# LockedFlysher/optimal_control_problem

Hardware: NVIDIA B200
Metric: batched OCP SQP solves/sec (H=20) (higher is better)
Workload: dtype f64

## Files before the change

optimal_control_problem_b200/csrc/admm_common.cuh:

```cuda
#pragma once

#include <cuda_runtime.h>
#include <stdint.h>
#include <stdio.h>

#include "ocp_b200.h"

namespace ocpb200 {

constexpr double kInfty = 1e30, kMinScaling = 1e-4, kMaxScaling = 1e4;
constexpr double kRhoMin = 1e-6, kRhoMax = 1e6, kRhoTol = 1e-4, kRhoEqOverIneq = 1e3;
constexpr double kDivisionTol = 1e-30;
constexpr int kRedWidth = 16;
constexpr int kMaxWarps = 32;

typedef uint16_t idx_t;

#ifdef OCP_B200_CANARY
constexpr int kCanaryDoubles = 2;
#else
constexpr int kCanaryDoubles = 0;
#endif
__device__ __forceinline__ double canary_value(int id) { return __longlong_as_double(0x7ff4dead00000000LL + id); }

struct KRun { uint16_t ka, kc, len, row0; };
struct KEntry {
  uint32_t dest0, dest1;
  int32_t ppos;
  uint32_t run_begin;
  uint16_t nruns, diag;
  uint32_t pad;
};

struct PatternDev {
  int n, m, nnz_a, nnz_p, nnz_h;
  int nblk, minv_doubles, max_bs;
  int n_long, n_short;
  int tri_ok, tri_np, tri_bs, tri_nb, tri_ld;
  int stage_slots;
  int kprog_entries;
  const KEntry* kprog;
  const KRun* kruns;
  int idx_entries;
  const idx_t* idx_base;
  const idx_t* a_colptr;
  const idx_t* a_rowidx;
  const idx_t* a_rowptr;
  const idx_t* a_colidx;
  const idx_t* a_perm;
  const idx_t* p_colptr;
  const idx_t* p_rowidx;
  const int* p_src;
  const idx_t* blk_ptr;
  const idx_t* blk_of_col;
  const int* minv_off;
  const idx_t* rows_long;
  const idx_t* rows_short;
};

struct SolveArgs {
  int B;
  const double* h_vals; int ld_h;
  const double* q; int ld_n;
  const double* a_vals; int ld_a;
  const double* l; const double* u; int ld_m;
  double* sol_x;
  double* sol_y;
  double* info;
  double* x_iter; int np; int N; double sqp_alpha;
  double* stats; int first_step;
  double* trace; int max_trace; int* n_trace;
  long long* phase;
  int* counter;
  double* slab; size_t slab_doubles;
};

struct Reducer {
  double* buf;
  int parity;
  int half;
};

template <int NV, bool kMax>
__device__ __forceinline__ void block_reduce(double (&v)[NV], Reducer& R) {
  const int lane = threadIdx.x & 31, warp = threadIdx.x >> 5, nw = blockDim.x >> 5;
#pragma unroll
  for (int k = 0; k < NV; ++k) {
    double a = v[k];
#pragma unroll
    for (int o = 16; o > 0; o >>= 1) {
      const double b = __shfl_xor_sync(0xffffffffu, a, o);
      a = kMax ? fmax(a, b) : a + b;
    }
    v[k] = a;
  }
  double* buf = R.buf + R.parity * R.half;
  R.parity ^= 1;
  if (lane == 0) {
#pragma unroll
    for (int k = 0; k < NV; ++k) buf[warp * NV + k] = v[k];
  }
  __syncthreads();
#pragma unroll
  for (int k = 0; k < NV; ++k) {
    double a = buf[k];
    for (int w = 1; w < nw; ++w) a = kMax ? fmax(a, buf[w * NV + k]) : a + buf[w * NV + k];
    v[k] = a;
  }
}

__device__ __forceinline__ double limit_scaling(double v) {
  v = v < kMinScaling ? 1.0 : v;
  return v > kMaxScaling ? kMaxScaling : v;
}

template <typename F>
__device__ __forceinline__ void for_rows_A(const PatternDev& P, const double* __restrict__ Aval,
                                           const double* __restrict__ src, F f) {
  const int tid = threadIdx.x, T = blockDim.x;
  for (int base = 0; base < P.n_long; base += (T >> 2)) {
    const int idx = base + (tid >> 2);
    const bool valid = idx < P.n_long;
    double s = 0.0;
    int row = 0;
    if (valid) {
      row = P.rows_long[idx];
      const int e = P.a_rowptr[row + 1];
#pragma unroll 4
      for (int k = P.a_rowptr[row] + (tid & 3); k < e; k += 4) s += Aval[P.a_perm[k]] * src[P.a_colidx[k]];
    }
    s += __shfl_xor_sync(0xffffffffu, s, 1);
    s += __shfl_xor_sync(0xffffffffu, s, 2);
    if (valid && (tid & 3) == 0) f(row, s);
  }
  for (int idx = tid; idx < P.n_short; idx += T) {
    const int row = P.rows_short[idx];
    double s = 0.0;
    const int e = P.a_rowptr[row + 1];
#pragma unroll 4
    for (int k = P.a_rowptr[row]; k < e; ++k) s += Aval[P.a_perm[k]] * src[P.a_colidx[k]];
    f(row, s);
  }
}

__device__ __forceinline__ double col_dot_A(const PatternDev& P, const double* __restrict__ Aval,
                                            const double* __restrict__ v, int j) {
  double s = 0.0;
  const int e = P.a_colptr[j + 1];
#pragma unroll 4
  for (int k = P.a_colptr[j]; k < e; ++k) s += Aval[k] * v[P.a_rowidx[k]];
  return s;
}
__device__ __forceinline__ double col_dot_P(const PatternDev& P, const double* __restrict__ Pval,
                                            const double* __restrict__ v, int j) {
  double s = 0.0;
  const int e = P.p_colptr[j + 1];
#pragma unroll 4
  for (int k = P.p_colptr[j]; k < e; ++k) s += Pval[k] * v[P.p_rowidx[k]];
  return s;
}

struct PhaseClock {
  long long* out; long long t0;
  __device__ PhaseClock(long long* o) : out((blockIdx.x == 0 && threadIdx.x == 0) ? o : nullptr), t0(0) { if (out) t0 = clock64(); }
  __device__ __forceinline__ void lap(int phase) {
    if (out) { const long long t = clock64(); out[phase] += t - t0; t0 = t; }
  }
};


#ifdef OCP_B200_FINE_PHASES
#define OCP_B200_FINE_CLOCK(name, ptr) PhaseClock name(ptr)
#define OCP_B200_FINE_LAP(name, phase) name.lap(phase)
#else
#define OCP_B200_FINE_CLOCK(name, ptr)
#define OCP_B200_FINE_LAP(name, phase)
#endif

struct QpResult {
  int status, iters, pcg_iters, rho_updates, checks;
  double prim_res, dual_res, rho;
};

__device__ inline void write_outputs(const PatternDev& P, const SolveArgs& A, const double* xs, const double* ys,
                                      Reducer& R, int inst, const QpResult& res) {
  const bool solved_setup = res.status != OCP_B200_QP_UNSOLVED || res.iters > 0;
  if (A.sol_x)
    for (int j = threadIdx.x; j < P.n; j += blockDim.x) A.sol_x[size_t(inst) * P.n + j] = solved_setup ? xs[j] : 0.0;
  if (A.sol_y)
    for (int i = threadIdx.x; i < P.m; i += blockDim.x) A.sol_y[size_t(inst) * P.m + i] = solved_setup ? ys[i] : 0.0;
  double nrm[1] = {0.0};
  if (A.x_iter) {
    double* xi = A.x_iter + size_t(inst) * A.N;
    for (int i = threadIdx.x; i < A.N; i += blockDim.x) {
      const double dx = solved_setup ? A.sqp_alpha * xs[A.np + i] : 0.0;
      xi[i] += dx;
      nrm[0] += dx * dx;
    }
    block_reduce<1, false>(nrm, R);
  }
  if (threadIdx.x == 0) {
    if (A.info) {
      double* f = A.info + size_t(inst) * OCP_B200_NINFO;
      f[OCP_B200_INFO_STATUS] = res.status; f[OCP_B200_INFO_ITERS] = res.iters;
      f[OCP_B200_INFO_PCG_ITERS] = res.pcg_iters; f[OCP_B200_INFO_PRIM_RES] = res.prim_res;
      f[OCP_B200_INFO_DUAL_RES] = res.dual_res; f[OCP_B200_INFO_RHO] = res.rho;
      f[OCP_B200_INFO_RHO_UPDATES] = res.rho_updates; f[OCP_B200_INFO_CHECKS] = res.checks;
    }
    if (A.stats) {
      double* s = A.stats + size_t(inst) * OCP_B200_NSTATS;
      if (A.first_step) for (int k = 0; k < OCP_B200_NSTATS; ++k) s[k] = 0.0;
      s[OCP_B200_STAT_QP_STATUS] = res.status;
      s[OCP_B200_STAT_SQP_STEPS] += 1.0;
      s[OCP_B200_STAT_ADMM_ITERS] += res.iters;
      s[OCP_B200_STAT_PCG_ITERS] += res.pcg_iters;
      s[OCP_B200_STAT_PRIM_RES] = res.prim_res;
      s[OCP_B200_STAT_DUAL_RES] = res.dual_res;
      s[OCP_B200_STAT_RHO_UPDATES] += res.rho_updates;
      s[OCP_B200_STAT_LAST_ADMM] = res.iters;
      s[OCP_B200_STAT_LAST_RHO] = res.rho;
      s[OCP_B200_STAT_CHECKS] += res.checks;
      s[OCP_B200_STAT_STEP_NORM] = sqrt(nrm[0]);
    }
  }
  __syncthreads();
}

}
```

optimal_control_problem_b200/csrc/admm_compact_kernel.cuh:

```cuda
#pragma once

#include "admm_direct_kernel.cuh"
#include "periodic_index.h"

namespace ocpb200 {
namespace compact {

using direct::Rho;
using direct::Work;

constexpr int kMaxGuards = 40;
struct Layout {
  int nguard;
  size_t guard_off[kMaxGuards];
  bool guard_slab[kMaxGuards];
  size_t b, x, w, z, y, vend;
  size_t aval, ctype, dp, xp, piv, arena, smem_doubles;
  size_t rscale, psm;
  size_t dp2, s, sp, stage, fb;
  int s_stride, sp_stride, stage_stride;
  size_t dinv, lsub, lp, q, l, u, D, E, pval, dx, dy, an, cn, sx, sz, sy, slab_doubles;
  bool ok, q_smem, lu_smem, scale_smem;
};

// ... 215 lines not shown
}

template <int BS>
__device__ inline void tri_solve_twisted_tmem(const PatternDev& P, const Work& W, uint32_t tmem) {
  const int tid = threadIdx.x, T = blockDim.x, lane = tid & 31, warp = tid >> 5;
  const int np = P.tri_np, nb = P.tri_nb, N = nb * BS;
  constexpr int ld = BS + 2;
  const int mid = nb / 2;
  double* bx = W.b + np;
  OCP_B200_FINE_CLOCK(clk, W.phase);
  const uint32_t base = tmem + (static_cast<uint32_t>(32 * (warp & 3)) << 16);
  double Lj[8];
  if (warp < 2) run_chain_tmem<BS, false>(W, bx, sweep_chain(warp, nb), base, lane);
  if (warp == 0 && mid + 1 < nb) slab_block_part<BS, false>(W.Lsub, mid + 1, lane, Lj);
  __syncthreads();
  if (warp == 0 && mid + 1 < nb) direct::sweep_stage<BS>(Lj, bx + (mid + 1) * BS + (lane & 1) * 8, bx + mid * BS + (lane >> 1), (lane & 1) == 0);
  __syncthreads();
  OCP_B200_FINE_LAP(clk, OCP_B200_PHASE_SOLVE_FWD);
  if (np > 0) {
    const int nw = T >> 5;
    if (direct::border_rows_by_warp(np, N, nw)) {
      direct::border_rows_dispatch(W.Lp, bx, W.b, W.xp, N, warp, lane, nw);
    } else {
    const int hw = tid >> 4, hl = tid & 15, nhw = T >> 4;
    for (int r0 = 0; r0 < np; r0 += nhw) {
      const int r = r0 + hw;
      const bool have = r < np;
      const double* rowp = W.Lp + size_t(have ? r : 0) * N;
      double s0 = 0.0, s1 = 0.0;
      for (int j0 = hl; j0 < N; j0 += 128) {
        double lv[8], yv[8];
#pragma unroll
        for (int u = 0; u < 8; ++u) {
          const int j = j0 + 16 * u;
          const bool ok = have && j < N;
          lv[u] = ok ? rowp[j] : 0.0;
          yv[u] = ok ? bx[j] : 0.0;
        }
#pragma unroll
        for (int u = 0; u < 8; u += 2) { s0 = fma(lv[u], yv[u], s0); s1 = fma(lv[u + 1], yv[u + 1], s1); }
      }
      double s = s0 + s1;
#pragma unroll
      for (int o = 8; o > 0; o >>= 1) s += __shfl_xor_sync(0xffffffffu, s, o);
      if (have && hl == 0) W.xp[r] = W.b[r] - s;
    }
    }
    __syncthreads();
    direct::border_apply_inverse(W.Dp, W.xp, W.b, np, tid);
    __syncthreads();
  }
  OCP_B200_FINE_LAP(clk, OCP_B200_PHASE_SOLVE_BORDER);
  {
#ifndef OCP_B200_DIAG_PASSES
#define OCP_B200_DIAG_PASSES 1
#endif
    constexpr int kPass = OCP_B200_DIAG_PASSES;
    const int Tb = (T / BS) * BS;
    const int k1 = tid / BS, r1 = tid % BS, kstep = T / BS;
    for (int base0 = 0, k0 = k1; base0 < N; base0 += kPass * Tb, k0 += kPass * kstep) {
      double vq[kPass];
#pragma unroll
      for (int q = 0; q < kPass; ++q) {
        const int base_j = base0 + q * Tb, k = k0 + q * kstep;
        const int j = tid < Tb ? base_j + tid : N;
        double v = 0.0;
        if (j < N) {
          {
            const double2* d2 = reinterpret_cast<const double2*>(W.Dinv + size_t(k) * BS * ld + r1 * ld);
            const double* yk = bx + k * BS;
            double dr[BS];
#pragma unroll
            for (int t = 0; t < BS / 2; ++t) { const double2 x = d2[t]; dr[2 * t] = x.x; dr[2 * t + 1] = x.y; }
            double s0 = 0.0, s1 = 0.0, s2 = 0.0, s3 = 0.0;
#pragma unroll
            for (int t = 0; t < BS; t += 4) {
              s0 = fma(dr[t], yk[t], s0); s1 = fma(dr[t + 1], yk[t + 1], s1);
              s2 = fma(dr[t + 2], yk[t + 2], s2); s3 = fma(dr[t + 3], yk[t + 3], s3);
            }
            v = (s0 + s1) + (s2 + s3);
          }
          double v1 = 0.0;
          if (np == 12) {
            double lv[12];
#pragma unroll
            for (int p = 0; p < 12; ++p) lv[p] = W.Lp[size_t(p) * N + j];
#pragma unroll
            for (int p = 0; p < 12; p += 2) { v = fma(-lv[p], W.b[p], v); v1 = fma(-lv[p + 1], W.b[p + 1], v1); }
          } else {
            int p = 0;
            for (; p + 1 < np; p += 2) {
              v = fma(-W.Lp[size_t(p) * N + j], W.b[p], v);
              v1 = fma(-W.Lp[size_t(p + 1) * N + j], W.b[p + 1], v1);
            }
            if (p < np) v = fma(-W.Lp[size_t(p) * N + j], W.b[p], v);
          }
          v += v1;
        }
        vq[q] = v;
      }
      __syncthreads();
#pragma unroll
      for (int q = 0; q < kPass; ++q) {
        const int j = tid < Tb ? base0 + q * Tb + tid : N;
        if (j < N) bx[j] = vq[q];
      }
    }
  }
  __syncthreads();
  OCP_B200_FINE_LAP(clk, OCP_B200_PHASE_SOLVE_DIAG);
  if (warp == 2 || warp == 3) run_chain_tmem<BS, true>(W, bx, sweep_chain(warp, nb), base, lane);
  __syncthreads();
  OCP_B200_FINE_LAP(clk, OCP_B200_PHASE_SOLVE_BWD);
}

template <int BS, bool kTile>
__device__ inline void solve_instance(const PatternDev& P, const CompactIdx& C, const ocp_b200_settings& S, const SolveArgs& A,
                                      Work& W, const Ctx& X, Reducer& R, int inst, QpResult& out, uint32_t tmem) {
  const int tid = threadIdx.x, T = blockDim.x;
  const int n = P.n, m = P.m;
  const double sigma = S.sigma, relax = S.relax;
  const uint32_t* const ar = X.ar;
  PhaseClock clk(A.phase);
  W.phase = A.phase;

  {
    const double* hv = A.h_vals + size_t(inst) * A.ld_h;
    const double* av = A.a_vals + size_t(inst) * A.ld_a;
    const double* qv = A.q + size_t(inst) * A.ld_n;
    const double* lv = A.l + size_t(inst) * A.ld_m;
    const double* uv = A.u + size_t(inst) * A.ld_m;
    for (int k = tid; k < P.nnz_a; k += T) W.Aval[k] = __ldcs(av + k);
    for (int k = tid; k < P.nnz_p; k += T) { const int s = P.p_src[k]; X.psm[k] = s >= 0 ? __ldcs(hv + s) : 0.0; }
    for (int j = tid; j < n; j += T) { W.q[j] = __ldcs(qv + j); W.D[j] = 1.0; }
    double bad[1] = {0.0};
    for (int i = tid; i < m; i += T) {
      const double lo = __ldcs(lv + i), hi = __ldcs(uv + i);
      if (lo > hi) bad[0] = 1.0;
      W.l[i] = fmax(lo, -kInfty);
      W.u[i] = fmin(hi, kInfty);
      W.E[i] = 1.0;
    }
    block_reduce<1, true>(bad, R);
    if (bad[0] > 0.0) {
      for (int j = tid; j < n; j += T) W.x[j] = 0.0;
      for (int i = tid; i < m; i += T) W.y[i] = 0.0;
      __syncthreads();
      out = QpResult{OCP_B200_QP_UNSOLVED, 0, 0, 0, 0, 0.0, 0.0, S.rho};
      return;
    }
  }
  clk.lap(OCP_B200_PHASE_LOAD);

  double c = 1.0;
  {
    const uint32_t* ta = ar + C.acol.tent_off;
    const uint32_t* tr2 = ar + C.arow.tent2_off;
    const uint32_t* tp = ar + C.pcol.tent_off;
    double* const cs = W.b;
    double* const rs = X.rscale;
    double* const Ps = X.psm;
    for (int pass = 0; pass < S.scaling_iters; ++pass) {
      for (int j = tid; j < n; j += T) {
        double dn = 0.0;
        if (pass == 0) {
          const PSpan sp = pspan_dev(C.pcol, ar, j);
#pragma unroll 4
          for (int kt = sp.kt0; kt < sp.kt1; ++kt) dn = fmax(dn, fabs(Ps[kt + sp.kshift]));
          const PSpan sa = pspan_dev(C.acol, ar, j);
#pragma unroll 4
          for (int kt = sa.kt0; kt < sa.kt1; ++kt) dn = fmax(dn, fabs(W.Aval[kt + sa.kshift]));
        } else {
          dn = fmax(X.cn[j], X.an[j]);
        }
        cs[j] = 1.0 / sqrt(limit_scaling(dn));
      }
      for (int i = tid; i < m; i += T) {
        const PSpan s = pspan_dev(C.arow, ar, i);
        double en = 0.0;
        if (s.qd2 >= 0) {
          const double* av = W.Aval + s.qd2;
#pragma unroll 4
          for (int kt = s.kt0; kt < s.kt1; ++kt) en = fmax(en, fabs(av[plow(tr2, kt)]));
        } else {
#pragma unroll 4
          for (int kt = s.kt0; kt < s.kt1; ++kt) en = fmax(en, fabs(W.Aval[pvalue(tr2[kt], s.q)]));
        }
        rs[i] = 1.0 / sqrt(limit_scaling(en));
      }
      __syncthreads();
      double red[2] = {0.0, 0.0};
      for (int j = tid; j < n; j += T) {
        const double dj = cs[j];
        const double q0 = W.q[j], d0 = W.D[j];
        double cn = 0.0, an = 0.0;
        const PSpan sp = pspan_dev(C.pcol, ar, j);
        for (int kt = sp.kt0; kt < sp.kt1; ++kt) {
          const double v = Ps[kt + sp.kshift] * cs[pvalue(tp[kt], sp.q)] * dj;
          Ps[kt + sp.kshift] = v;
          cn = fmax(cn, fabs(v));
        }
        const PSpan sa = pspan_dev(C.acol, ar, j);
#pragma unroll 4
        for (int kt = sa.kt0; kt < sa.kt1; ++kt) {
          const double v = W.Aval[kt + sa.kshift] * (rs[pvalue(ta[kt], sa.q)] * dj);
          W.Aval[kt + sa.kshift] = v;
          an = fmax(an, fabs(v));
        }
        X.an[j] = an;
        X.cn[j] = cn;
        const double qj = q0 * dj;
        W.q[j] = qj;
        W.D[j] = d0 * dj;
        red[0] += cn;
        red[1] = fmax(red[1], fabs(qj));
      }
      for (int i = tid; i < m; i += T) W.E[i] *= rs[i];
      double sum[1] = {red[0]}, mx[1] = {red[1]};
      block_reduce<1, false>(sum, R);
      block_reduce<1, true>(mx, R);
      const double ct = 1.0 / limit_scaling(fmax(sum[0] / double(n), limit_scaling(mx[0])));
      for (int k = tid; k < P.nnz_p; k += T) Ps[k] *= ct;
      for (int j = tid; j < n; j += T) { W.q[j] *= ct; X.cn[j] *= ct; }
      c *= ct;
      __syncthreads();
    }
  }
  const double cinv = 1.0 / c;

  double rho = fmin(fmax(S.rho, kRhoMin), kRhoMax);
  for (int i = tid; i < m; i += T) {
    const double e = W.E[i];
    const double lo = W.l[i] * e, hi = W.u[i] * e;
    W.l[i] = lo; W.u[i] = hi;
    signed char ct = 0;
    if (lo < -kInfty * kMinScaling && hi > kInfty * kMinScaling) ct = -1;
    else if (hi - lo < kRhoTol) ct = 1;
    W.ctype[i] = ct;
  }
  for (int k = tid; k < P.nnz_p; k += T) X.pslab[k] = X.psm[k];
  __syncthreads();
  W.Pval = X.pslab;
  Rho rv(rho);
  clk.lap(OCP_B200_PHASE_SCALE);
  direct::tri_assemble_program(P, W, rv, sigma);
  clk.lap(OCP_B200_PHASE_KKT_ASSEMBLE);
  direct::tri_factor_twisted<BS, true, kTile>(P, W);
  if constexpr (BS == 16) tmem_publish<BS>(W, P.tri_nb, tmem);
  clk.lap(OCP_B200_PHASE_FACTOR);
  for (int j = tid; j < n; j += T) W.x[j] = 0.0;
  for (int i = tid; i < m; i += T) { W.z[i] = 0.0; W.y[i] = 0.0; W.w[i] = 0.0; }
  __syncthreads();

  const int rho_interval = S.adaptive_rho_interval > 0 ? S.adaptive_rho_interval : (S.check_termination > 0 ? 4 * S.check_termination : 100);
  int status = OCP_B200_QP_UNSOLVED, iter = 0, solves = 0, rho_updates = 0, checks = 0, n_trace = 0;
  double prim_res = 0.0, dual_res = 0.0;
  bool done = false;

  for (iter = 1; iter <= S.admm_max_iter && !done; ++iter) {
    for (int j = tid; j < n; j += T) {
      const double qj = W.q[j];
      W.b[j] = (sigma * W.x[j] - qj) + col_dot_A(C, ar, W.Aval, W.w, j);
    }
    __syncthreads();
    clk.lap(OCP_B200_PHASE_RHS);
    if constexpr (BS == 16) tri_solve_twisted_tmem<BS>(P, W, tmem);
    else direct::tri_solve_twisted<BS>(P, W);
    ++solves;
    clk.lap(OCP_B200_PHASE_SOLVE);

    const bool can_check = S.check_termination > 0 && (iter % S.check_termination == 0);
    const bool last_iter = iter == S.admm_max_iter;
    const bool rho_time = S.adaptive_rho && rho_interval > 0 && (iter % rho_interval == 0);
    const bool want_info = can_check || rho_time || last_iter;
    {
      const uint32_t* tc = ar + C.arow.tent_off;
      const uint32_t* tp = ar + C.arow.tent2_off;
      for (int i = tid; i < m; i += T) {
        const double lo = W.l[i], hi = W.u[i];
        const PSpan s = pspan_dev(C.arow, ar, i);
        double zt = 0.0;
        if (s.qd >= 0 && s.qd2 >= 0) {
          const double* av = W.Aval + s.qd2;
          const double* bv = W.b + s.qd;
#pragma unroll 4
          for (int kt = s.kt0; kt < s.kt1; ++kt) zt += av[plow(tp, kt)] * bv[plow(tc, kt)];
        } else {
#pragma unroll 4
          for (int kt = s.kt0; kt < s.kt1; ++kt) zt += W.Aval[pvalue(tp[kt], s.q)] * W.b[pvalue(tc[kt], s.q)];
        }
        const signed char ct = W.ctype[i];
        const double rh = rv.of(ct);
        const double zr = relax * zt + (1.0 - relax) * W.z[i];
        const double zn = fmin(fmax(zr + rv.inv(ct) * W.y[i], lo), hi);
        const double dy = rh * (zr - zn);
        const double yn = W.y[i] + dy;
        W.y[i] = yn;
        W.z[i] = zn;
        W.w[i] = rh * zn - yn;
        if (want_info) W.dy[i] = dy;
      }
    }
    for (int j = tid; j < n; j += T) {
      const double xo = W.x[j];
      const double xn = relax * W.b[j] + (1.0 - relax) * xo;
      if (want_info) W.dx[j] = xn - xo;
      W.x[j] = xn;
    }
    __syncthreads();
    clk.lap(OCP_B200_PHASE_UPDATE);
    if (!want_info) continue;

    ++checks;
    double mx[kRedWidth];
#pragma unroll
    for (int k = 0; k < kRedWidth; ++k) mx[k] = 0.0;
    for_rows_A(C, ar, m, W.Aval, W.x, [&](int i, double ax) {
      const double einv = 1.0 / W.E[i];
      const double zi = W.z[i];
      const double rp = ax - zi;
      mx[0] = fmax(mx[0], fabs(einv * rp));
      mx[1] = fmax(mx[1], fabs(einv * ax));
      mx[2] = fmax(mx[2], fabs(einv * zi));
      mx[3] = fmax(mx[3], fabs(rp));
      mx[4] = fmax(mx[4], fabs(ax));
      mx[5] = fmax(mx[5], fabs(zi));
    });
    for (int j = tid; j < n; j += T) {
      const double dinv = 1.0 / W.D[j];
      const double qj = W.q[j];
      const double px = col_dot_P(C, ar, W.Pval, W.x, j);
      const double aty = col_dot_A(C, ar, W.Aval, W.y, j);
      const double rd = qj + px + aty;
      mx[6] = fmax(mx[6], fabs(dinv * rd));
      mx[7] = fmax(mx[7], fabs(dinv * qj));
      mx[8] = fmax(mx[8], fabs(dinv * px));
      mx[9] = fmax(mx[9], fabs(dinv * aty));
      mx[10] = fmax(mx[10], fabs(rd));
      mx[11] = fmax(mx[11], fabs(qj));
      mx[12] = fmax(mx[12], fabs(px));
      mx[13] = fmax(mx[13], fabs(aty));
    }
    block_reduce<kRedWidth, true>(mx, R);
    prim_res = mx[0];
    dual_res = cinv * mx[6];

    if (can_check || last_iter) {
      const double eps_prim = S.eps_abs + S.eps_rel * fmax(mx[2], mx[1]);
      const double eps_dual = S.eps_abs + S.eps_rel * cinv * fmax(mx[7], fmax(mx[9], mx[8]));
      const bool prim_ok = prim_res < eps_prim, dual_ok = dual_res < eps_dual;
      bool prim_inf = false, dual_inf = false;
      if (!prim_ok) {
        double a2[1] = {0.0};
        for (int i = tid; i < m; i += T) {
          double dy = W.dy[i];
          const double lo = W.l[i], hi = W.u[i];
          if (hi > kInfty * kMinScaling) {
            if (lo < -kInfty * kMinScaling) dy = 0.0; else dy = fmin(dy, 0.0);
          } else if (lo < -kInfty * kMinScaling) {
            dy = fmax(dy, 0.0);
          }
          W.dy[i] = dy;
          a2[0] = fmax(a2[0], fabs(W.E[i] * dy));
        }
        block_reduce<1, true>(a2, R);
        const double norm_dy = a2[0];
        if (norm_dy > kDivisionTol) {
          double lhs[1] = {0.0};
          for (int i = tid; i < m; i += T) lhs[0] += W.u[i] * fmax(W.dy[i], 0.0) + W.l[i] * fmin(W.dy[i], 0.0);
          block_reduce<1, false>(lhs, R);
          if (lhs[0] < -S.eps_prim_inf * norm_dy) {
            __syncthreads();
            double na[1] = {0.0};
            for (int j = tid; j < n; j += T) na[0] = fmax(na[0], fabs(col_dot_A(C, ar, W.Aval, W.dy, j) / W.D[j]));
            block_reduce<1, true>(na, R);
            prim_inf = na[0] < S.eps_prim_inf * norm_dy;
          }
        }
      }
      if (!dual_ok) {
        double a2[1] = {0.0};
        for (int j = tid; j < n; j += T) a2[0] = fmax(a2[0], fabs(W.D[j] * W.dx[j]));
        block_reduce<1, true>(a2, R);
        const double norm_dx = a2[0];
        if (norm_dx > kDivisionTol) {
          double qdx[1] = {0.0};
          for (int j = tid; j < n; j += T) qdx[0] += W.q[j] * W.dx[j];
          block_reduce<1, false>(qdx, R);
          if (qdx[0] < -c * S.eps_dual_inf * norm_dx) {
            double np_[1] = {0.0};
            for (int j = tid; j < n; j += T) np_[0] = fmax(np_[0], fabs(col_dot_P(C, ar, W.Pval, W.dx, j) / W.D[j]));
            block_reduce<1, true>(np_, R);
            if (np_[0] < c * S.eps_dual_inf * norm_dx) {
// ... 144 lines not shown
```

optimal_control_problem_b200/csrc/tri_fast.cuh:

```cuda
#pragma once

namespace ocpb200 {
namespace direct {

template <int BS> struct TriCfg {
  static constexpr int LPR = BS <= 8 ? 4 : (BS <= 16 ? 2 : 1);
  static constexpr int CPL = BS / LPR;
  static_assert(BS % LPR == 0 && CPL % 2 == 0, "block size must split into even lane chunks");
};

template <int BS>
__device__ __forceinline__ double dot_cc(const double* __restrict__ a, const double* __restrict__ b) {
  const double2* a2 = reinterpret_cast<const double2*>(a);
  const double2* b2 = reinterpret_cast<const double2*>(b);
  double s0 = 0.0, s1 = 0.0, s2 = 0.0, s3 = 0.0;
#pragma unroll
  for (int t = 0; t < BS / 2; t += 2) {
    const double2 x0 = a2[t], y0 = b2[t];
    s0 = fma(x0.x, y0.x, s0); s1 = fma(x0.y, y0.y, s1);
    if (t + 1 < BS / 2) {
      const double2 x1 = a2[t + 1], y1 = b2[t + 1];
      s2 = fma(x1.x, y1.x, s2); s3 = fma(x1.y, y1.y, s3);
    }
  }
  return (s0 + s1) + (s2 + s3);
}

template <int BS>
__device__ __forceinline__ double dot_cs(const double* __restrict__ a, const double* __restrict__ b, int sb) {
  const double2* a2 = reinterpret_cast<const double2*>(a);
  double s0 = 0.0, s1 = 0.0, s2 = 0.0, s3 = 0.0;
#pragma unroll
  for (int t = 0; t < BS / 2; t += 2) {
    const double2 x0 = a2[t];
    s0 = fma(x0.x, b[(2 * t) * sb], s0); s1 = fma(x0.y, b[(2 * t + 1) * sb], s1);
    if (t + 1 < BS / 2) {
      const double2 x1 = a2[t + 1];
      s2 = fma(x1.x, b[(2 * t + 2) * sb], s2); s3 = fma(x1.y, b[(2 * t + 3) * sb], s3);
    }
  }
  return (s0 + s1) + (s2 + s3);
}

template <int BS>
__device__ __forceinline__ void tile_cc(const double* __restrict__ a0, const double* __restrict__ a1,
                                        const double* __restrict__ b0, const double* __restrict__ b1, double (&o)[4]) {
  const double2* A0 = reinterpret_cast<const double2*>(a0);
  const double2* A1 = reinterpret_cast<const double2*>(a1);
  const double2* B0 = reinterpret_cast<const double2*>(b0);
  const double2* B1 = reinterpret_cast<const double2*>(b1);
  double s[4][4];
#pragma unroll
  for (int i = 0; i < 4; ++i) { s[i][0] = 0.0; s[i][1] = 0.0; s[i][2] = 0.0; s[i][3] = 0.0; }
#pragma unroll 2
  for (int t = 0; t < BS / 2; ++t) {
    const double2 x0 = A0[t], x1 = A1[t], y0 = B0[t], y1 = B1[t];
    const int k = (t & 1) * 2;
    s[0][k] = fma(x0.x, y0.x, s[0][k]); s[0][k + 1] = fma(x0.y, y0.y, s[0][k + 1]);
    s[1][k] = fma(x0.x, y1.x, s[1][k]); s[1][k + 1] = fma(x0.y, y1.y, s[1][k + 1]);
    s[2][k] = fma(x1.x, y0.x, s[2][k]); s[2][k + 1] = fma(x1.y, y0.y, s[2][k + 1]);
    s[3][k] = fma(x1.x, y1.x, s[3][k]); s[3][k + 1] = fma(x1.y, y1.y, s[3][k + 1]);
  }
#pragma unroll
  for (int i = 0; i < 4; ++i) o[i] = (s[i][0] + s[i][1]) + (s[i][2] + s[i][3]);
}
template <int BS>
__device__ __forceinline__ void tile_cs(const double* __restrict__ a0, const double* __restrict__ a1,
                                        const double* __restrict__ bcol, int sb, double (&o)[4]) {
  const double2* A0 = reinterpret_cast<const double2*>(a0);
  const double2* A1 = reinterpret_cast<const double2*>(a1);
  double s[4][4];
#pragma unroll
  for (int i = 0; i < 4; ++i) { s[i][0] = 0.0; s[i][1] = 0.0; s[i][2] = 0.0; s[i][3] = 0.0; }
#pragma unroll 2
  for (int t = 0; t < BS / 2; ++t) {
    const double2 x0 = A0[t], x1 = A1[t];
    const double2 ya = *reinterpret_cast<const double2*>(bcol + (2 * t) * sb);
    const double2 yb = *reinterpret_cast<const double2*>(bcol + (2 * t + 1) * sb);
    const int k = (t & 1) * 2;
    s[0][k] = fma(x0.x, ya.x, s[0][k]); s[0][k + 1] = fma(x0.y, yb.x, s[0][k + 1]);
    s[1][k] = fma(x0.x, ya.y, s[1][k]); s[1][k + 1] = fma(x0.y, yb.y, s[1][k + 1]);
    s[2][k] = fma(x1.x, ya.x, s[2][k]); s[2][k + 1] = fma(x1.y, yb.x, s[2][k + 1]);
    s[3][k] = fma(x1.x, ya.y, s[3][k]); s[3][k + 1] = fma(x1.y, yb.y, s[3][k + 1]);
  }
#pragma unroll
  for (int i = 0; i < 4; ++i) o[i] = (s[i][0] + s[i][1]) + (s[i][2] + s[i][3]);
}

template <int BS, int LD = BS + 2>
__device__ __forceinline__ void warp_invert_exact(double* M, int , int lane, double* piv) {
  constexpr int ld = LD;
  static_assert(BS % 2 == 0 && BS <= 32, "one column per lane, even size");
  const bool act = lane < BS;
  const int cc = act ? lane : 0;
  double col[BS];
#pragma unroll
  for (int r = 0; r < BS; ++r) col[r] = M[r * ld + cc];
  const double2* piv2 = reinterpret_cast<const double2*>(piv);
  double rnext = 1.0 / col[0];
#pragma unroll
  for (int k = 0; k < BS; ++k) {
    const double ck = col[k];
    const double ipiv = __shfl_sync(0xffffffffu, rnext, k);
    const bool mine = lane == k;
    const double fl = mine ? ipiv : (lane < k ? ck * ipiv : -ck * ipiv);
    if (act) piv[lane] = fl;
    if (k + 1 < BS) rnext = 1.0 / fma(fl, ck, col[k + 1 < BS ? k + 1 : k]);
    __syncwarp();
#pragma unroll
    for (int r = 0; r < BS / 2; ++r) {
      const double2 f = piv2[r];
      const int r0 = 2 * r, r1 = 2 * r + 1;
      col[r0] = mine ? f.x : (r0 == k ? ck * f.x : fma(f.x, ck, col[r0]));
      col[r1] = mine ? f.y : (r1 == k ? ck * f.y : fma(f.y, ck, col[r1]));
    }
    __syncwarp();
  }
  if (act) {
#pragma unroll
    for (int r = 0; r < BS; ++r) M[r * ld + lane] = col[r];
  }
}

__device__ __forceinline__ void invert_border(double* Dp, int np, int lane, double* piv) {
  if (np == 12) warp_invert_exact<12, 13>(Dp, 13, lane, piv);
  else if (np == 4) warp_invert_exact<4, 5>(Dp, 5, lane, piv);
  else if (np == 24) warp_invert_exact<24, 25>(Dp, 25, lane, piv);
  else warp_invert(Dp, np, np + 1, lane);
}

template <int BS>
__device__ __forceinline__ void sweep_stage(const double (&Lpart)[TriCfg<BS>::CPL], const double* __restrict__ src,
                                            double* __restrict__ dst, bool writer) {
  constexpr int CPL = TriCfg<BS>::CPL, LPR = TriCfg<BS>::LPR;
  const double old = writer ? *dst : 0.0;
  double s0 = 0.0, s1 = 0.0, s2 = 0.0, s3 = 0.0;
#pragma unroll
  for (int c = 0; c < CPL; c += 4) {
    s0 = fma(Lpart[c], src[c], s0);
    s1 = fma(Lpart[c + 1], src[c + 1], s1);
    if (c + 2 < CPL) { s2 = fma(Lpart[c + 2], src[c + 2], s2); s3 = fma(Lpart[c + 3], src[c + 3], s3); }
  }
  double s = (s0 + s1) + (s2 + s3);
  if (LPR >= 2) s += __shfl_xor_sync(0xffffffffu, s, 1);
  if (LPR >= 4) s += __shfl_xor_sync(0xffffffffu, s, 2);
  if (writer) *dst = old - s;
  __syncwarp();
}

}
}
```

optimal_control_problem_b200/csrc/tri_twisted.cuh:

```cuda
#pragma once

namespace ocpb200 {
namespace direct {

__device__ __forceinline__ void group_barrier(int id, int nthreads) {
  asm volatile("bar.sync %0, %1;" ::"r"(id), "r"(nthreads) : "memory");
}

template <int BS, bool kTop, bool kStaged = false, bool kTile = false>
__device__ __forceinline__ void chain_step(const Work& W, int np, int N, int , int k, int pred, int slot, double* S,
                                           double* Sp, double* Dpacc, int gt, int GT, int bar, double* stage, double* F = nullptr) {
  constexpr int bb = BS * BS, ld = BS + 2;
  const int pb = np * BS;
  double* Cg = W.Lsub + size_t(slot) * BS * ld;
  double* Dk = W.Dinv + size_t(k) * BS * ld;
  const double* Dg = W.Dinv + size_t(pred) * BS * ld;
  const double* C = Cg;
  const double* Dm = Dg;
  if (kStaged || stage != nullptr) {
    double2* cs = reinterpret_cast<double2*>(stage);
    double2* ds = reinterpret_cast<double2*>(stage + W.stage_stride);
    const double2* cg2 = reinterpret_cast<const double2*>(Cg);
    const double2* dg2 = reinterpret_cast<const double2*>(Dg);
    for (int e = gt; e < BS * ld / 2; e += GT) { cs[e] = cg2[e]; ds[e] = dg2[e]; }
    group_barrier(bar, GT);
    C = stage; Dm = stage + W.stage_stride;
  }
  if constexpr (kTile) {
    for (int e = gt; e < bb / 4; e += GT) {
      const int r0 = 2 * (e / (BS / 2)), c0 = 2 * (e % (BS / 2));
      double o[4];
      if (kTop) {
        tile_cc<BS>(C + r0 * ld, C + (r0 + 1) * ld, Dm + c0 * ld, Dm + (c0 + 1) * ld, o);
        S[r0 * ld + c0] = o[0]; S[r0 * ld + c0 + 1] = o[1]; S[(r0 + 1) * ld + c0] = o[2]; S[(r0 + 1) * ld + c0 + 1] = o[3];
      } else {
        tile_cs<BS>(Dm + c0 * ld, Dm + (c0 + 1) * ld, C + r0, ld, o);
        S[r0 * ld + c0] = o[0]; S[(r0 + 1) * ld + c0] = o[1]; S[r0 * ld + c0 + 1] = o[2]; S[(r0 + 1) * ld + c0 + 1] = o[3];
      }
    }
  } else {
  for (int e = gt; e < bb; e += GT) {
    const int r = e / BS, c = e % BS;
    S[r * ld + c] = kTop ? dot_cc<BS>(C + r * ld, Dm + c * ld) : dot_cs<BS>(Dm + c * ld, C + r, ld);
  }
  }
  for (int e = gt; e < pb; e += GT) {
    const int r = e / BS, c = e % BS;
    Sp[e] = W.Lp[size_t(r) * N + pred * BS + c];
  }
  group_barrier(bar, GT);
  const bool tile_p = kTile && (np & 1) == 0;
  if constexpr (kTile) {
    for (int e = gt; e < bb / 4; e += GT) {
      const int r0 = 2 * (e / (BS / 2)), c0 = 2 * (e % (BS / 2));
      double o[4];
      if (kTop) tile_cc<BS>(S + r0 * ld, S + (r0 + 1) * ld, C + c0 * ld, C + (c0 + 1) * ld, o);
      else tile_cs<BS>(S + r0 * ld, S + (r0 + 1) * ld, C + c0, ld, o);
      Dk[r0 * ld + c0] -= o[0]; Dk[r0 * ld + c0 + 1] -= o[1]; Dk[(r0 + 1) * ld + c0] -= o[2]; Dk[(r0 + 1) * ld + c0 + 1] -= o[3];
    }
  } else {
  for (int e = gt; e < bb; e += GT) {
    const int r = e / BS, c = e % BS;
    Dk[r * ld + c] -= kTop ? dot_cc<BS>(S + r * ld, C + c * ld) : dot_cs<BS>(S + r * ld, C + c, ld);
  }
  }
  if (tile_p) {
    for (int e = gt; e < pb / 4; e += GT) {
      const int r0 = 2 * (e / (BS / 2)), c0 = 2 * (e % (BS / 2));
      double so[4], fo[4];
      tile_cc<BS>(Sp + r0 * BS, Sp + (r0 + 1) * BS, S + c0 * ld, S + (c0 + 1) * ld, so);
      tile_cc<BS>(Sp + r0 * BS, Sp + (r0 + 1) * BS, Dm + c0 * ld, Dm + (c0 + 1) * ld, fo);
#pragma unroll
      for (int i = 0; i < 2; ++i)
#pragma unroll
        for (int j = 0; j < 2; ++j) {
          const int r = r0 + i, c = c0 + j;
          W.Lp[size_t(r) * N + k * BS + c] -= so[2 * i + j];
          W.Lp[size_t(r) * N + pred * BS + c] = fo[2 * i + j];
          if (kStaged || F != nullptr) F[r * BS + c] = fo[2 * i + j];
        }
    }
  } else {
  for (int e = gt; e < pb; e += GT) {
    const int r = e / BS, c = e % BS;
    const double s = dot_cc<BS>(Sp + r * BS, S + c * ld);
    const double f = dot_cc<BS>(Sp + r * BS, Dm + c * ld);
    W.Lp[size_t(r) * N + k * BS + c] -= s;
    W.Lp[size_t(r) * N + pred * BS + c] = f;
    if (kStaged || F != nullptr) F[e] = f;
  }
  }
  group_barrier(bar, GT);
  if (tile_p && (kStaged || F != nullptr)) {
    const int hp = np / 2;
    for (int e = gt; e < hp * hp; e += GT) {
      const int r0 = 2 * (e / hp), c0 = 2 * (e - (e / hp) * hp);
      double o[4];
      tile_cc<BS>(Sp + r0 * BS, Sp + (r0 + 1) * BS, F + c0 * BS, F + (c0 + 1) * BS, o);
      Dpacc[r0 * (np + 1) + c0] += o[0]; Dpacc[r0 * (np + 1) + c0 + 1] += o[1];
      Dpacc[(r0 + 1) * (np + 1) + c0] += o[2]; Dpacc[(r0 + 1) * (np + 1) + c0 + 1] += o[3];
    }
  } else {
  for (int e = gt; e < np * np; e += GT) {
    const int r = e / np, c = e - r * np;
    Dpacc[r * (np + 1) + c] += (kStaged || F != nullptr) ? dot_cc<BS>(Sp + r * BS, F + c * BS)
                                            : dot_cs<BS>(Sp + r * BS, W.Lp + size_t(c) * N + pred * BS, 1);
  }
  }
  for (int e = gt; e < bb; e += GT) {
    const int r = e / BS, c = e % BS;
    Cg[r * ld + c] = S[r * ld + c];
  }
  group_barrier(bar, GT);
}

template <int BS, bool kStaged = false, bool kTile = false>
__device__ inline void tri_factor_twisted(const PatternDev& P, const Work& W) {
  const int tid = threadIdx.x, T = blockDim.x, lane = tid & 31;
  const int np = P.tri_np, nb = P.tri_nb, N = nb * BS;
  constexpr int ld = BS + 2;
  const int mid = nb / 2;
  const int GT = T / 2;
  const int grp = tid >= GT ? 1 : 0, gt = tid - grp * GT;
  double* S = W.S + grp * W.s_stride;
  double* Sp = W.Sp + grp * W.sp_stride;
  double* piv = W.piv + grp * 32;
  double* Dpacc = W.Dp2 + grp * np * (np + 1);
  double* stage = (kStaged || W.stage) ? W.stage + grp * 2 * W.stage_stride : nullptr;
  double* F = (kStaged || W.Fb) ? W.Fb + grp * W.sp_stride : nullptr;
  for (int e = gt; e < np * (np + 1); e += GT) Dpacc[e] = 0.0;
  if (grp == 0) {
    OCP_B200_FINE_CLOCK(clk, W.phase);
    for (int k = 0; k < mid; ++k) {
      if (gt < 32) warp_invert_exact<BS>(W.Dinv + size_t(k) * BS * ld, ld, lane, piv);
      group_barrier(1, GT);
      OCP_B200_FINE_LAP(clk, OCP_B200_PHASE_FACTOR_INVERT);
      chain_step<BS, true, kStaged, kTile>(W, np, N, ld, k + 1, k, k + 1, S, Sp, Dpacc, gt, GT, 1, stage, F);
      OCP_B200_FINE_LAP(clk, OCP_B200_PHASE_FACTOR_STEP);
    }
  } else {
    for (int k = nb - 1; k > mid + 1; --k) {
      if (gt < 32) warp_invert_exact<BS>(W.Dinv + size_t(k) * BS * ld, ld, lane, piv);
      group_barrier(2, GT);
      chain_step<BS, false, kStaged, kTile>(W, np, N, ld, k - 1, k, k, S, Sp, Dpacc, gt, GT, 2, stage, F);
    }
    if (mid + 1 < nb) {
      if (gt < 32) warp_invert_exact<BS>(W.Dinv + size_t(mid + 1) * BS * ld, ld, lane, piv);
      group_barrier(2, GT);
    }
  }
  __syncthreads();
  if (mid + 1 < nb) chain_step<BS, false, kStaged, kTile>(W, np, N, ld, mid, mid + 1, mid + 1, W.S, W.Sp, W.Dp2, tid, T, 0, W.stage, W.Fb);
  if (tid < 32) warp_invert_exact<BS>(W.Dinv + size_t(mid) * BS * ld, ld, lane, W.piv);
  __syncthreads();
  if (np > 0) {
    const double* Dm = W.Dinv + size_t(mid) * BS * ld;
    const int pb = np * BS;
    for (int e = tid; e < pb; e += T) {
      const int r = e / BS, c = e % BS;
      W.Sp[e] = W.Lp[size_t(r) * N + mid * BS + c];
    }
    __syncthreads();
    for (int e = tid; e < pb; e += T) {
      const int r = e / BS, c = e % BS;
      const double f = dot_cc<BS>(W.Sp + r * BS, Dm + c * ld);
      W.Lp[size_t(r) * N + mid * BS + c] = f;
      if (kStaged || W.Fb != nullptr) W.Fb[e] = f;
    }
    __syncthreads();
    for (int e = tid; e < np * np; e += T) {
      const int r = e / np, c = e - r * np;
      const int o = r * (np + 1) + c;
      W.Dp[o] -= W.Dp2[o] + W.Dp2[np * (np + 1) + o] +
                 ((kStaged || W.Fb != nullptr) ? dot_cc<BS>(W.Sp + r * BS, W.Fb + c * BS)
                                  : dot_cs<BS>(W.Sp + r * BS, W.Lp + size_t(c) * N + mid * BS, 1));
    }
    __syncthreads();
    if (tid < 32) invert_border(W.Dp, np, lane, W.piv);
    __syncthreads();
  }
}

template <int BS, bool kColumn>
__device__ __forceinline__ void ring_stage(const double* __restrict__ blk, const double* __restrict__ src,
                                           double* __restrict__ dst, bool writer, bool src_vec) {
  constexpr int ld = BS + 2;
  static_assert(TriCfg<BS>::LPR == 1 && BS % 4 == 0, "one lane per row");
  double lv[BS], sv[BS];
  if (!kColumn) {
    const double2* p2 = reinterpret_cast<const double2*>(blk);
#pragma unroll
    for (int i = 0; i < BS / 2; ++i) { const double2 v = p2[i]; lv[2 * i] = v.x; lv[2 * i + 1] = v.y; }
  } else {
#pragma unroll
    for (int i = 0; i < BS; ++i) lv[i] = blk[i * ld];
  }
  if (src_vec) {
    const double2* q2 = reinterpret_cast<const double2*>(src);
#pragma unroll
    for (int i = 0; i < BS / 2; ++i) { const double2 v = q2[i]; sv[2 * i] = v.x; sv[2 * i + 1] = v.y; }
  } else {
#pragma unroll
    for (int i = 0; i < BS; ++i) sv[i] = src[i];
  }
  const double old = writer ? *dst : 0.0;
  double s0 = 0.0, s1 = 0.0, s2 = 0.0, s3 = 0.0;
#pragma unroll
  for (int c = 0; c < BS; c += 4) {
    s0 = fma(lv[c], sv[c], s0); s1 = fma(lv[c + 1], sv[c + 1], s1);
    s2 = fma(lv[c + 2], sv[c + 2], s2); s3 = fma(lv[c + 3], sv[c + 3], s3);
  }
  if (writer) *dst = old - ((s0 + s1) + (s2 + s3));
  __syncwarp();
}

template <int BS, bool kColumn>
__device__ __forceinline__ void run_chain(const Work& W, double* bx, int , int slot0, int dslot, int dst0, int src0,
                                          int dblk, int count, int lane, int chain) {
  constexpr int CPL = TriCfg<BS>::CPL, LPR = TriCfg<BS>::LPR, ld = BS + 2;
  const int row = lane / LPR, half = lane % LPR;
  const bool act = row < BS;
  const int rr = act ? row : 0;
  const bool writer = act && half == 0;
  if (count <= 0) return;
  const double* lp = W.Lsub + size_t(slot0) * BS * ld + (kColumn ? size_t(half * CPL) * ld + rr : size_t(rr) * ld + half * CPL);
  const int dl = dslot * BS * ld, db = dblk * BS;
  const double* srcp = bx + src0 * BS + half * CPL;
  double* dstp = bx + dst0 * BS + rr;
  auto load = [&](double (&dst)[CPL], const double* p) {
    if (!kColumn) {
      const double2* p2 = reinterpret_cast<const double2*>(p);
#pragma unroll
      for (int i = 0; i < CPL / 2; ++i) { const double2 v = p2[i]; dst[2 * i] = v.x; dst[2 * i + 1] = v.y; }
    } else {
#pragma unroll
      for (int i = 0; i < CPL; ++i) dst[i] = p[i * ld];
    }
  };
  if constexpr (CPL > 8) if (W.ring_slots >= 2) {
    const int R = W.ring_slots, stride = W.stage_stride;
    double* ring = W.stage + chain * R * stride;
    unsigned long long* bars = W.ring_bar + chain * kMaxRing;
    constexpr uint32_t bytes = BS * ld * sizeof(double);
    const double* gp = W.Lsub + size_t(slot0) * BS * ld;
    uint32_t ph = W.ring_phase[chain];
    if (lane == 0)
      for (int i = 0; i < R && i < count; ++i) ring_issue(ring + i * stride, gp + i * dl, bytes, bars + i);
    const int off = kColumn ? (half * CPL) * ld + rr : rr * ld + half * CPL;
    const bool src_vec = (reinterpret_cast<unsigned long long>(srcp) & 15ULL) == 0ULL;
    int s = 0;
    for (int i = 0; i < count; ++i) {
      ring_wait(bars + s, (ph >> s) & 1u);
      ph ^= 1u << s;
      ring_stage<BS, kColumn>(ring + s * stride + off, srcp, dstp, writer, src_vec);
      if (lane == 0 && i + R < count) ring_issue(ring + s * stride, gp + (i + R) * dl, bytes, bars + s);
      srcp += db; dstp += db;
      s = s + 1 == R ? 0 : s + 1;
    }
    if (lane == 0) W.ring_phase[chain] = ph;
    __syncwarp();
    return;
  }
  if (W.stage != nullptr && CPL <= 8) {
    double La[CPL], Lb[CPL], Lc[CPL];
    load(La, lp);
    if (count > 1) load(Lb, lp + dl);
    for (int i = 0; i < count; i += 3) {
      if (i + 2 < count) load(Lc, lp + 2 * dl);
      sweep_stage<BS>(La, srcp, dstp, writer);
      if (i + 1 < count) {
        if (i + 3 < count) load(La, lp + 3 * dl);
        sweep_stage<BS>(Lb, srcp + db, dstp + db, writer);
      }
      if (i + 2 < count) {
        if (i + 4 < count) load(Lb, lp + 4 * dl);
        sweep_stage<BS>(Lc, srcp + 2 * db, dstp + 2 * db, writer);
      }
      lp += 3 * dl; srcp += 3 * db; dstp += 3 * db;
    }
    return;
  }
  double La[CPL], Lb[CPL];
  load(La, lp);
  for (int i = 0; i < count; i += 2) {
    if (i + 1 < count) load(Lb, lp + dl);
    sweep_stage<BS>(La, srcp, dstp, writer);
    if (i + 1 < count) {
      if (i + 2 < count) load(La, lp + 2 * dl);
      sweep_stage<BS>(Lb, srcp + db, dstp + db, writer);
    }
    lp += 2 * dl; srcp += 2 * db; dstp += 2 * db;
  }
}

template <int RW, bool kExact>
__device__ __forceinline__ void border_rows_warp(const double* __restrict__ Lp, const double* __restrict__ y,
                                                 const double* __restrict__ bp, double* __restrict__ xp, int N, int warp,
                                                 int lane) {
  constexpr int U = 10;
  double lv[RW][U];
#pragma unroll
  for (int r = 0; r < RW; ++r) {
    const double* rowp = Lp + size_t(warp * RW + r) * N;
#pragma unroll
    for (int u = 0; u < U; ++u) {
      const int j = lane + 32 * u;
      const double v = rowp[kExact || j < N ? j : N - 1];
      lv[r][u] = kExact || j < N ? v : 0.0;
    }
// ... 175 lines not shown
```

Measured before the change: 58630.

## Overlap block inversion with async staging and fuse scaling reductions

In the staged twisted tridiagonal factorization, the non-inverting warps now prefetch the next sub-diagonal block and Lp slice into shared memory with cp.async while warp 0 inverts the diagonal block. The inverse is also written directly into the stage buffer, so chain_step skips its own copy. Separately, the Ruiz scaling loop merges the sum and max block reductions into one pass and applies the cost scale lazily in the next iteration instead of sweeping P and q separately. The added complexity covers stage-buffer aliasing (a third stage region is used for the middle step) and the assumption that GT exceeds 32 threads.

```diff
diff --git a/optimal_control_problem_b200/csrc/admm_common.cuh b/optimal_control_problem_b200/csrc/admm_common.cuh
--- a/optimal_control_problem_b200/csrc/admm_common.cuh
+++ b/optimal_control_problem_b200/csrc/admm_common.cuh
@@ -109,6 +109,23 @@
   }
 }
 
+__device__ __forceinline__ void block_reduce_sum_max(double& sum, double& mx, Reducer& R) {
+  const int lane = threadIdx.x & 31, warp = threadIdx.x >> 5, nw = blockDim.x >> 5;
+  double a = sum, b = mx;
+#pragma unroll
+  for (int o = 16; o > 0; o >>= 1) {
+    a += __shfl_xor_sync(0xffffffffu, a, o);
+    b = fmax(b, __shfl_xor_sync(0xffffffffu, b, o));
+  }
+  double* buf = R.buf + R.parity * R.half;
+  R.parity ^= 1;
+  if (lane == 0) { buf[2 * warp] = a; buf[2 * warp + 1] = b; }
+  __syncthreads();
+  a = buf[0]; b = buf[1];
+  for (int w = 1; w < nw; ++w) { a += buf[2 * w]; b = fmax(b, buf[2 * w + 1]); }
+  sum = a; mx = b;
+}
+
 __device__ __forceinline__ double limit_scaling(double v) {
   v = v < kMinScaling ? 1.0 : v;
   return v > kMaxScaling ? kMaxScaling : v;
diff --git a/optimal_control_problem_b200/csrc/admm_compact_kernel.cuh b/optimal_control_problem_b200/csrc/admm_compact_kernel.cuh
--- a/optimal_control_problem_b200/csrc/admm_compact_kernel.cuh
+++ b/optimal_control_problem_b200/csrc/admm_compact_kernel.cuh
@@ -391,7 +391,7 @@
   }
   clk.lap(OCP_B200_PHASE_LOAD);
 
-  double c = 1.0;
+  double c = 1.0, cf = 1.0;
   {
     const uint32_t* ta = ar + C.acol.tent_off;
     const uint32_t* tr2 = ar + C.arow.tent2_off;
@@ -410,7 +410,7 @@
 #pragma unroll 4
           for (int kt = sa.kt0; kt < sa.kt1; ++kt) dn = fmax(dn, fabs(W.Aval[kt + sa.kshift]));
         } else {
-          dn = fmax(X.cn[j], X.an[j]);
+          dn = fmax(X.cn[j] * cf, X.an[j]);
         }
         cs[j] = 1.0 / sqrt(limit_scaling(dn));
       }
@@ -425,17 +425,19 @@
 #pragma unroll 4
           for (int kt = s.kt0; kt < s.kt1; ++kt) en = fmax(en, fabs(W.Aval[pvalue(tr2[kt], s.q)]));
         }
-        rs[i] = 1.0 / sqrt(limit_scaling(en));
+        const double r = 1.0 / sqrt(limit_scaling(en));
+        rs[i] = r;
+        W.E[i] *= r;
       }
       __syncthreads();
       double red[2] = {0.0, 0.0};
       for (int j = tid; j < n; j += T) {
         const double dj = cs[j];
-        const double q0 = W.q[j], d0 = W.D[j];
+        const double q0 = W.q[j] * cf, d0 = W.D[j];
         double cn = 0.0, an = 0.0;
         const PSpan sp = pspan_dev(C.pcol, ar, j);
         for (int kt = sp.kt0; kt < sp.kt1; ++kt) {
-          const double v = Ps[kt + sp.kshift] * cs[pvalue(tp[kt], sp.q)] * dj;
+          const double v = Ps[kt + sp.kshift] * cf * cs[pvalue(tp[kt], sp.q)] * dj;
           Ps[kt + sp.kshift] = v;
           cn = fmax(cn, fabs(v));
         }
@@ -454,15 +456,9 @@
         red[0] += cn;
         red[1] = fmax(red[1], fabs(qj));
       }
-      for (int i = tid; i < m; i += T) W.E[i] *= rs[i];
-      double sum[1] = {red[0]}, mx[1] = {red[1]};
-      block_reduce<1, false>(sum, R);
-      block_reduce<1, true>(mx, R);
-      const double ct = 1.0 / limit_scaling(fmax(sum[0] / double(n), limit_scaling(mx[0])));
-      for (int k = tid; k < P.nnz_p; k += T) Ps[k] *= ct;
-      for (int j = tid; j < n; j += T) { W.q[j] *= ct; X.cn[j] *= ct; }
-      c *= ct;
-      __syncthreads();
+      block_reduce_sum_max(red[0], red[1], R);
+      cf = 1.0 / limit_scaling(fmax(red[0] / double(n), limit_scaling(red[1])));
+      c *= cf;
     }
   }
   const double cinv = 1.0 / c;
@@ -477,7 +473,8 @@
     else if (hi - lo < kRhoTol) ct = 1;
     W.ctype[i] = ct;
   }
-  for (int k = tid; k < P.nnz_p; k += T) X.pslab[k] = X.psm[k];
+  for (int k = tid; k < P.nnz_p; k += T) X.pslab[k] = X.psm[k] * cf;
+  for (int j = tid; j < n; j += T) W.q[j] *= cf;
   __syncthreads();
   W.Pval = X.pslab;
   Rho rv(rho);
diff --git a/optimal_control_problem_b200/csrc/tri_fast.cuh b/optimal_control_problem_b200/csrc/tri_fast.cuh
--- a/optimal_control_problem_b200/csrc/tri_fast.cuh
+++ b/optimal_control_problem_b200/csrc/tri_fast.cuh
@@ -88,7 +88,7 @@
 }
 
 template <int BS, int LD = BS + 2>
-__device__ __forceinline__ void warp_invert_exact(double* M, int , int lane, double* piv) {
+__device__ __forceinline__ void warp_invert_exact(double* M, int , int lane, double* piv, double* M2 = nullptr) {
   constexpr int ld = LD;
   static_assert(BS % 2 == 0 && BS <= 32, "one column per lane, even size");
   const bool act = lane < BS;
@@ -119,6 +119,10 @@
   if (act) {
 #pragma unroll
     for (int r = 0; r < BS; ++r) M[r * ld + lane] = col[r];
+    if (M2 != nullptr) {
+#pragma unroll
+      for (int r = 0; r < BS; ++r) M2[r * ld + lane] = col[r];
+    }
   }
 }
 
diff --git a/optimal_control_problem_b200/csrc/tri_twisted.cuh b/optimal_control_problem_b200/csrc/tri_twisted.cuh
--- a/optimal_control_problem_b200/csrc/tri_twisted.cuh
+++ b/optimal_control_problem_b200/csrc/tri_twisted.cuh
@@ -6,6 +6,12 @@
 __device__ __forceinline__ void group_barrier(int id, int nthreads) {
   asm volatile("bar.sync %0, %1;" ::"r"(id), "r"(nthreads) : "memory");
 }
+
+__device__ __forceinline__ void cp_async16(double* dst, const double* src) {
+  asm volatile("cp.async.cg.shared.global [%0], [%1], 16;" ::"r"(static_cast<uint32_t>(__cvta_generic_to_shared(dst))),
+               "l"(src) : "memory");
+}
+__device__ __forceinline__ void cp_async_wait_all() { asm volatile("cp.async.wait_all;" ::: "memory"); }
 
 template <int BS, bool kTop, bool kStaged = false, bool kTile = false>
 __device__ __forceinline__ void chain_step(const Work& W, int np, int N, int , int k, int pred, int slot, double* S,
@@ -15,9 +21,9 @@
   double* Cg = W.Lsub + size_t(slot) * BS * ld;
   double* Dk = W.Dinv + size_t(k) * BS * ld;
   const double* Dg = W.Dinv + size_t(pred) * BS * ld;
-  const double* C = Cg;
-  const double* Dm = Dg;
-  if (kStaged || stage != nullptr) {
+  const double* C = kStaged ? stage : Cg;
+  const double* Dm = kStaged ? stage + W.stage_stride : Dg;
+  if (!kStaged && stage != nullptr) {
     double2* cs = reinterpret_cast<double2*>(stage);
     double2* ds = reinterpret_cast<double2*>(stage + W.stage_stride);
     const double2* cg2 = reinterpret_cast<const double2*>(Cg);
@@ -44,9 +50,11 @@
     S[r * ld + c] = kTop ? dot_cc<BS>(C + r * ld, Dm + c * ld) : dot_cs<BS>(Dm + c * ld, C + r, ld);
   }
   }
-  for (int e = gt; e < pb; e += GT) {
-    const int r = e / BS, c = e % BS;
-    Sp[e] = W.Lp[size_t(r) * N + pred * BS + c];
+  if (!kStaged) {
+    for (int e = gt; e < pb; e += GT) {
+      const int r = e / BS, c = e % BS;
+      Sp[e] = W.Lp[size_t(r) * N + pred * BS + c];
+    }
   }
   group_barrier(bar, GT);
   const bool tile_p = kTile && (np & 1) == 0;
@@ -129,32 +137,79 @@
   double* stage = (kStaged || W.stage) ? W.stage + grp * 2 * W.stage_stride : nullptr;
   double* F = (kStaged || W.Fb) ? W.Fb + grp * W.sp_stride : nullptr;
   for (int e = gt; e < np * (np + 1); e += GT) Dpacc[e] = 0.0;
-  if (grp == 0) {
-    OCP_B200_FINE_CLOCK(clk, W.phase);
-    for (int k = 0; k < mid; ++k) {
-      if (gt < 32) warp_invert_exact<BS>(W.Dinv + size_t(k) * BS * ld, ld, lane, piv);
-      group_barrier(1, GT);
-      OCP_B200_FINE_LAP(clk, OCP_B200_PHASE_FACTOR_INVERT);
-      chain_step<BS, true, kStaged, kTile>(W, np, N, ld, k + 1, k, k + 1, S, Sp, Dpacc, gt, GT, 1, stage, F);
-      OCP_B200_FINE_LAP(clk, OCP_B200_PHASE_FACTOR_STEP);
-    }
-  } else {
-    for (int k = nb - 1; k > mid + 1; --k) {
-      if (gt < 32) warp_invert_exact<BS>(W.Dinv + size_t(k) * BS * ld, ld, lane, piv);
-      group_barrier(2, GT);
-      chain_step<BS, false, kStaged, kTile>(W, np, N, ld, k - 1, k, k, S, Sp, Dpacc, gt, GT, 2, stage, F);
-    }
-    if (mid + 1 < nb) {
-      if (gt < 32) warp_invert_exact<BS>(W.Dinv + size_t(mid + 1) * BS * ld, ld, lane, piv);
-      group_barrier(2, GT);
-    }
-  }
-  __syncthreads();
-  if (mid + 1 < nb) chain_step<BS, false, kStaged, kTile>(W, np, N, ld, mid, mid + 1, mid + 1, W.S, W.Sp, W.Dp2, tid, T, 0, W.stage, W.Fb);
-  if (tid < 32) warp_invert_exact<BS>(W.Dinv + size_t(mid) * BS * ld, ld, lane, W.piv);
-  __syncthreads();
+  const double* Dmid = W.Dinv + size_t(mid) * BS * ld;
+  if constexpr (kStaged) {
+    double* Dm = stage + W.stage_stride;
+    auto fetch = [&](int slot, int vblk) {
+      const int lt = gt - 32, NL = GT - 32;
+      const double* cg = W.Lsub + size_t(slot) * BS * ld;
+#pragma unroll 1
+      for (int e = lt; e < BS * ld / 2; e += NL) cp_async16(stage + 2 * e, cg + 2 * e);
+#pragma unroll 1
+      for (int e = lt; e < np * BS / 2; e += NL) {
+        const int r = 2 * e / BS, c = 2 * e - r * BS;
+        cp_async16(Sp + 2 * e, W.Lp + size_t(r) * N + vblk * BS + c);
+      }
+      cp_async_wait_all();
+    };
+    if (grp == 0) {
+      OCP_B200_FINE_CLOCK(clk, W.phase);
+      for (int k = 0; k < mid; ++k) {
+        if (gt < 32) warp_invert_exact<BS>(W.Dinv + size_t(k) * BS * ld, ld, lane, piv, Dm);
+        else fetch(k + 1, k);
+        group_barrier(1, GT);
+        OCP_B200_FINE_LAP(clk, OCP_B200_PHASE_FACTOR_INVERT);
+        chain_step<BS, true, true, kTile>(W, np, N, ld, k + 1, k, k + 1, S, Sp, Dpacc, gt, GT, 1, stage, F);
+        OCP_B200_FINE_LAP(clk, OCP_B200_PHASE_FACTOR_STEP);
+      }
+    } else {
+      for (int k = nb - 1; k > mid + 1; --k) {
+        if (gt < 32) warp_invert_exact<BS>(W.Dinv + size_t(k) * BS * ld, ld, lane, piv, Dm);
+        else fetch(k, k);
+        group_barrier(2, GT);
+        chain_step<BS, false, true, kTile>(W, np, N, ld, k - 1, k, k, S, Sp, Dpacc, gt, GT, 2, stage, F);
+      }
+      if (mid + 1 < nb) {
+        if (gt < 32) warp_invert_exact<BS>(W.Dinv + size_t(mid + 1) * BS * ld, ld, lane, piv, Dm);
+        else fetch(mid + 1, mid + 1);
+        group_barrier(2, GT);
+      }
+    }
+    __syncthreads();
+    double* const bstage = W.stage + 2 * W.stage_stride;
+    if (mid + 1 < nb) chain_step<BS, false, true, kTile>(W, np, N, ld, mid, mid + 1, mid + 1, W.S, W.Sp + W.sp_stride, W.Dp2, tid, T, 0, bstage, W.Fb);
+    double* const Dtop = W.stage + W.stage_stride;
+    if (tid < 32) warp_invert_exact<BS>(W.Dinv + size_t(mid) * BS * ld, ld, lane, W.piv, Dtop);
+    __syncthreads();
+    Dmid = Dtop;
+  } else {
+    if (grp == 0) {
+      OCP_B200_FINE_CLOCK(clk, W.phase);
+      for (int k = 0; k < mid; ++k) {
+        if (gt < 32) warp_invert_exact<BS>(W.Dinv + size_t(k) * BS * ld, ld, lane, piv);
+        group_barrier(1, GT);
+        OCP_B200_FINE_LAP(clk, OCP_B200_PHASE_FACTOR_INVERT);
+        chain_step<BS, true, kStaged, kTile>(W, np, N, ld, k + 1, k, k + 1, S, Sp, Dpacc, gt, GT, 1, stage, F);
+        OCP_B200_FINE_LAP(clk, OCP_B200_PHASE_FACTOR_STEP);
+      }
+    } else {
+      for (int k = nb - 1; k > mid + 1; --k) {
+        if (gt < 32) warp_invert_exact<BS>(W.Dinv + size_t(k) * BS * ld, ld, lane, piv);
+        group_barrier(2, GT);
+        chain_step<BS, false, kStaged, kTile>(W, np, N, ld, k - 1, k, k, S, Sp, Dpacc, gt, GT, 2, stage, F);
+      }
+      if (mid + 1 < nb) {
+        if (gt < 32) warp_invert_exact<BS>(W.Dinv + size_t(mid + 1) * BS * ld, ld, lane, piv);
+        group_barrier(2, GT);
+      }
+    }
+    __syncthreads();
+    if (mid + 1 < nb) chain_step<BS, false, kStaged, kTile>(W, np, N, ld, mid, mid + 1, mid + 1, W.S, W.Sp, W.Dp2, tid, T, 0, W.stage, W.Fb);
+    if (tid < 32) warp_invert_exact<BS>(W.Dinv + size_t(mid) * BS * ld, ld, lane, W.piv);
+    __syncthreads();
+  }
   if (np > 0) {
-    const double* Dm = W.Dinv + size_t(mid) * BS * ld;
+    const double* Dm = Dmid;
     const int pb = np * BS;
     for (int e = tid; e < pb; e += T) {
       const int r = e / BS, c = e % BS;
```

After: 60900, median of 6. 3.9% higher.
